# AdityaNG/Low-Cost-Hardware-Accelerated-Vision-Based-Depth-Perception-for-Real-Time-Applications

Hardware: AMD Instinct MI355X
Metric: stereo pairs/sec, KITTI 1242x375 D=128 (ms/frame at batch 1 in latency_ms_batch1) (higher is better)
Workload: dtype u8; 1 GPU; kitti_1242x375_D128_batch256_per_gpu_streamed; width=1242, height=375, disp_max=127, preset=driver(MIDDLEBURY+only_left+adaptive_mean+median), parallelism=batch-sharded x1, no data-path collective

## Files before the change

low-cost-hardware-accelerated-vision-based-depth-perception-for-real-time-applications_amd/csrc/kernels.hip:

```cpp
#include "sv_kernels.h"
#include "wave_ops.h"

#include <algorithm>
#include <atomic>

namespace sv {

thread_local LaunchHook g_launch_hook = {nullptr, nullptr};

const char *kernel_name(int id) {
    static const char *names[K_COUNT] = {"descriptor", "support_match", "support_filter", "grid_mark", "grid_dilate", "plane_fit", "triangles_raster", "dense_match", "lr_check",
                                         "delaunay_gpu", "ccl_band", "ccl_finish", "gap_rows", "gap_cols", "adaptive_mean", "median", "output"};
    return (id >= 0 && id < K_COUNT) ? names[id] : "?";
}



__device__ __forceinline__ uint32_t sad4(uint32_t a, uint32_t b, uint32_t acc) { return __builtin_amdgcn_sad_u8(a, b, acc); }

__device__ __forceinline__ uint32_t sad16(const uint4 &a, const uint4 &b) {
    uint32_t s = sad4(a.x, b.x, 0u);
    s = sad4(a.y, b.y, s);
    s = sad4(a.z, b.z, s);
    return sad4(a.w, b.w, s);
// ... 1127 lines not shown
        for (int r = 0; r < 3; r++) {
            A[r][0] = sd == 0 ? (double)pu[r] : (double)(pu[r] - pd[r]);
            A[r][1] = (double)pv[r];
            A[r][2] = 1.0;
            B[r] = (double)pd[r];
        }
        const bool ok = solve3(A, B);
        pl[3 * sd + 0] = ok ? (float)B[0] : 0.f;
        pl[3 * sd + 1] = ok ? (float)B[1] : 0.f;
        pl[3 * sd + 2] = ok ? (float)B[2] : 0.f;
    }
    const float plane_a = side == 0 ? pl[0] : pl[3], plane_b = side == 0 ? pl[1] : pl[4], plane_c = side == 0 ? pl[2] : pl[5];
    const float plane_d = side == 0 ? pl[3] : pl[0];
    const bool valid = (double)fabsf(plane_a) < 0.7 && (double)fabsf(plane_d) < 0.7;
    trirec[tbase] = make_float4(plane_a, plane_b, plane_c, valid ? 1.0f : 0.0f);
#pragma unroll
    for (int j = 0; j < 6; j++) planes[tbase * 6 + j] = pl[j];
    float tu[3], tv[3];
#pragma unroll
    for (int c = 0; c < 3; c++) {
        tu[c] = side == 0 ? (float)pu[c] : (float)(pu[c] - pd[c]);
        tv[c] = (float)pv[c];
    }
#pragma unroll
    for (int j = 0; j < 3; j++)
#pragma unroll
        for (int kk = 0; kk < j; kk++)
            if (tu[kk] > tu[j]) {
                float x = tu[j];
                tu[j] = tu[kk];
                tu[kk] = x;
                x = tv[j];
                tv[j] = tv[kk];
                tv[kk] = x;
            }
    const float A_u = tu[0], A_v = tv[0], B_u = tu[1], B_v = tv[1], C_u = tu[2], C_v = tv[2];
    float AB_a = 0, AC_a = 0, BC_a = 0;
    if ((int)A_u != (int)B_u) AB_a = (A_v - B_v) / (A_u - B_u);
    if ((int)A_u != (int)C_u) AC_a = (A_v - C_v) / (A_u - C_u);
    if ((int)B_u != (int)C_u) BC_a = (B_v - C_v) / (B_u - C_u);
    RasterRec r;
    r.a_u = (int)A_u;
    r.b_u = (int)B_u;
    r.c_u = (int)C_u;
    r.ac_a = AC_a;
    r.ac_b = A_v - AC_a * A_u;
    r.ab_a = AB_a;
    r.ab_b = A_v - AB_a * A_u;
    r.bc_a = BC_a;
    r.bc_b = B_v - BC_a * B_u;
    rrec[tbase] = r;
    ub = max(r.a_u, 0), ue = min(r.c_u, d.W);
    const float vlo = fminf(fminf(A_v, B_v), C_v), vhi = fmaxf(fmaxf(A_v, B_v), C_v);
    vb = max((int)vlo - 1, 0), ve = min((int)vhi + 2, d.H);
    }
    const bool bins = ub < ue && vb < ve;
    const int tx_lo = ub / RT_W, tx_hi = bins ? (ue - 1) / RT_W : -1, ty_lo = vb / RT_H, ty_hi = bins ? (ve - 1) / RT_H : -1;
    for (int ty = ty_lo; ty <= ty_hi; ty++)
        for (int tx = tx_lo; tx <= tx_hi; tx++) atomicAdd(&s_cnt[ty * ntx + tx], 1);
    __syncthreads();
    const size_t tb = (size_t)(pair * 2 + side) * ntile;
    for (int i = threadIdx.x; i < ntile; i += 256) {
        const int c = s_cnt[i];
        if (c > 0) s_base[i] = atomicAdd(&tile_cnt[tb + i], c);
        s_cnt[i] = 0;
    }
    __syncthreads();
    for (int ty = ty_lo; ty <= ty_hi; ty++)
        for (int tx = tx_lo; tx <= tx_hi; tx++) {
            const int tile = ty * ntx + tx;
            const int slot = s_base[tile] + atomicAdd(&s_cnt[tile], 1);
            if (slot < k.rt_cap) tile_list[(tb + tile) * RT_CAP + slot] = t;
        }
}


__global__ __launch_bounds__(256) void k_raster_tiles(KParams k, const int32_t *__restrict__ blob, const RasterRec *__restrict__ rrec, const int32_t *__restrict__ tile_cnt,
                                                      const int32_t *__restrict__ tile_list, int32_t *__restrict__ tri_id) {
    const Dims &d = k.d;
    const int pair = blockIdx.z, side = blockIdx.y;
    if (blob[pair * META_WORDS] < 3) return;
    const int ntx = (d.W + RT_W - 1) / RT_W;
    const int tx0 = (blockIdx.x % ntx) * RT_W, ty0 = (blockIdx.x / ntx) * RT_H;
    __shared__ int32_t tile[RT_H][RT_W];
    for (int i = threadIdx.x; i < RT_H * RT_W; i += 256) (&tile[0][0])[i] = -1;
    __syncthreads();
    const size_t gt = (size_t)(pair * 2 + side) * gridDim.x + blockIdx.x;
    const int listed = tile_cnt[gt];
    const bool all = listed > k.rt_cap;
    const int cnt = all ? blob[pair * META_WORDS + 2 + 2 * side] : listed;
    const int sub = threadIdx.x & 7, grp = threadIdx.x >> 3;
    const int x_end = min(tx0 + RT_W, d.W), y_end = min(ty0 + RT_H, d.H);
    const RasterRec *recs = rrec + (size_t)(pair * 2 + side) * d.max_tri;
    const int32_t *list = tile_list + gt * RT_CAP;
    int t_next = grp < cnt ? (all ? grp : list[grp]) : 0;
    RasterRec r_next = recs[t_next];
    for (int i = grp; i < cnt; i += 32) {
        const int t = t_next;
        const RasterRec r = r_next;
        if (i + 32 < cnt) {
            t_next = all ? i + 32 : list[i + 32];
            r_next = recs[t_next];
        }
        const int u_begin = max(max(r.a_u, 0), tx0), u_end = min(min(r.c_u, d.W), x_end);
        for (int base = u_begin; base < u_end; base += 8) {
            const int u = base + sub;
            int lo = 0x7FFFFFFF, hi = -0x7FFFFFFF;
            if (u < u_end) {
                const bool second = u >= r.b_u;
                const float e_a = second ? r.bc_a : r.ab_a, e_b = second ? r.bc_b : r.ab_b;
                const int v_1 = (int)(r.ac_a * (float)u + r.ac_b), v_2 = (int)(e_a * (float)u + e_b);
                lo = max(max(min(v_1, v_2), 0), ty0);
                hi = min(min(max(v_1, v_2), d.H), y_end);
                if (lo >= hi) {
                    lo = 0x7FFFFFFF;
                    hi = -0x7FFFFFFF;
                }
            }
            int32_t *p = lo < hi ? &tile[lo - ty0][u - tx0] : nullptr;
            for (int v = lo; v < hi; v++, p += RT_W) atomicMax(p, t);
        }
    }
    __syncthreads();
    int32_t *ids = tri_id + (size_t)(pair * 2 + side) * d.N;
    for (int i = threadIdx.x; i < RT_H * RT_W; i += 256) {
        const int r = i / RT_W, c = i - r * RT_W;
        if (ty0 + r < d.H && tx0 + c < d.W) map_st(ids, (uint32_t)((ty0 + r) * d.W + tx0 + c), tile[r][c]);
    }
}

void launch_triangles(const KParams &k, const SlotDev &s, int n, int max_points, hipStream_t st) {
    const int ntile = ((k.d.W + RT_W - 1) / RT_W) * ((k.d.H + RT_H - 1) / RT_H);
    const int nt = std::max(1, std::min(2 * max_points, k.d.max_tri));
    const size_t pl_lds = sizeof(int32_t) * 2 * (size_t)ntile;
    static std::atomic<size_t> pl_granted[64];
    ensure_dynamic_lds(k_planes, pl_lds, pl_granted, "plane_fit");
    SV_LAUNCH(K_PLANES, k_planes, dim3((nt + 255) / 256, 2, n), dim3(256), pl_lds, st, k, s.blob, s.trirec, s.planes, (RasterRec *)s.rrec, s.tile_cnt, s.tile_list);
    SV_LAUNCH(K_TRIANGLES, k_raster_tiles, dim3(ntile, 2, n), dim3(256), 0, st, k, s.blob, (const RasterRec *)s.rrec, s.tile_cnt, s.tile_list, s.tri_id);
}

#define DENSE_TW 512
#define DENSE_MASK_WORDS 8

template <int R>
__device__ __forceinline__ int dense_band_full(const KParams &k, int side, const uint4 own, const uint4 *pb, uint32_t vmask) {
    uint4 c[2 * R + 1];
#pragma unroll
    for (int s = 0; s <= 2 * R; s++) c[s] = pb[s];
    int key[2 * R + 1];
#pragma unroll
    for (int s = 0; s <= 2 * R; s++) {
        const int o = side ? s : 2 * R - s, ao = s < R ? R - s : s - R;
        key[s] = sad16_key(own, c[s], (int)(vmask & (((uint32_t)k.prior[ao] << 16) | (uint32_t)o)));
    }
    int bb = key[0];
#pragma unroll
    for (int s = 1; s + 1 <= 2 * R; s += 2) bb = min(bb, min(key[s], key[s + 1]));
    return bb;
}

template <bool COUNT, int MWT, int RT, bool TEX>
__device__ __forceinline__ int dense_pixel(const KParams &k, int side, int u, int v, const uint4 own, const uint4 *pu, const float4 rec, const uint32_t *mw,
                                             const uint32_t *cell, int &ncand, int (&npath)[5], const uint4 *lds_first, const uint4 *lds_last) {
    const Dims &d = k.d;
    const int MW = MWT ? MWT : d.MW, plane_radius = RT ? RT : k.plane_radius;
    if (TEX && (int)texture16(own) < k.match_texture) return -10;
    const int d_plane = (int)(rec.x * (float)u + rec.y * (float)v + rec.z);
    const int d_plane_min = max(d_plane - plane_radius, 0);
    const int d_plane_max = min(d_plane + plane_radius, d.D - 1);
    const bool valid = rec.w != 0.0f;
    const int a_lo = side ? 0 : max(u - (d.W - 3), 0), a_hi = side ? min(d.W - 3 - u, d.D - 1) : min(u - 2, d.D - 1);
    const int sgn = side ? 1 : -1;
    constexpr int KEY_NONE = 0x7FFF0000;
    int best = KEY_NONE;
    const int b_lo = max(d_plane_min, a_lo), b_hi = min(d_plane_max, a_hi);
    const bool clip = __builtin_amdgcn_ballot_w64(a_lo != 0 || a_hi != d.D - 1) != 0;
    const int band_bits = max(d_plane_max - d_plane_min + 1, 0), band_word = d_plane_min >> 5;
    const uint64_t band = (uint64_t)((1u << band_bits) - 1u) << (d_plane_min & 31);
    const uint32_t band_lo = (uint32_t)band, band_hi = (uint32_t)(band >> 32);
    uint32_t mc[DENSE_MASK_WORDS];
#pragma unroll
    for (int w = 0; w < DENSE_MASK_WORDS; w++) mc[w] = mw[w];
    if (clip) {
#pragma unroll
        for (int w = 0; w < DENSE_MASK_WORDS; w++) {
            if (w >= MW) break;
            const int lo = a_lo - 32 * w, hi = a_hi - 32 * w;
            uint32_t keep = 0;
            if (lo <= 31 && hi >= 0 && lo <= hi) {
                const int l = max(lo, 0), h = min(hi, 31);
                keep = (h == 31 ? 0xFFFFFFFFu : ((1u << (h + 1)) - 1u)) & ~((1u << l) - 1u);
            }
            mc[w] &= keep;
        }
    }
#pragma unroll
    for (int w = 0; w < DENSE_MASK_WORDS; w++) {
        if (w >= MW) break;
        if (__builtin_amdgcn_ballot_w64(mc[w] != 0u) == 0) continue;
        uint32_t m = mc[w] & ~(w == band_word ? band_lo : (w == band_word + 1 ? band_hi : 0u));
        if (COUNT) ncand += __popc(m);
        int best_w = KEY_NONE;
        while (m) {
            if (COUNT) {
                const unsigned long long act = __ballot(1);
                npath[3] += ((int)(threadIdx.x & 63) == __ffsll((long long)act) - 1) ? 1 : 0;
                npath[4]++;
            }
            const int b1 = __ffs((int)m) - 1;
            m &= m - 1;
// ... 151 lines not shown
                if (COUNT) npix++;
            }
            if (!d.sub)
                wta[(size_t)ps * d.N + (size_t)v * d.W + u] = (int16_t)out;
            else if (!(u & 1) && (u >> 1) < d.Wm && (v >> 1) < d.Hm)
                wta[(size_t)ps * d.Nm + (size_t)(v >> 1) * d.Wm + (u >> 1)] = (int16_t)out;
        }
    }
    if (COUNT) {
        count_add(counters + CNT_DENSE_CANDIDATES, ncand);
        count_add(counters + CNT_DENSE_PIXELS, npix);
        count_add(counters + CNT_DENSE_BAND_FULL, npath[0]);
        count_add(counters + CNT_DENSE_BAND_PART, npath[1]);
        count_add(counters + CNT_DENSE_BAND_SLOW, npath[2]);
        count_add(counters + CNT_DENSE_GRID_WAVE_TRIPS, npath[3]);
        count_add(counters + CNT_DENSE_GRID_LANE_TRIPS, npath[4]);
    }
}

static size_t dense_lds_bytes(const KParams &k) { return sizeof(uint4) * 2 * (size_t)dense_seg(k.d); }

template <int MWT, int RT, bool TEX>
static void launch_dense_as(const KParams &k, const SlotDev &s, const dim3 &grid, size_t shmem, hipStream_t st) {
    static std::atomic<size_t> granted[64];
    ensure_dynamic_lds(k_dense<false, MWT, RT, TEX>, shmem, granted, "dense_match");
    SV_LAUNCH(K_DENSE, (k_dense<false, MWT, RT, TEX>), grid, dim3(256), shmem, st, k, s.grad, s.blob, s.tri_id, s.trirec, s.gmaskB, s.wta, s.counters);
}

void launch_dense(const KParams &k, const SlotDev &s, int n, hipStream_t st) {
    const size_t shmem = dense_lds_bytes(k);
    const dim3 grid((k.d.W + DENSE_TW - 1) / DENSE_TW, k.d.sub ? (k.d.H + 1) / 2 : k.d.H, n);
    if (s.counters) {
        static std::atomic<size_t> granted_c[64];
        ensure_dynamic_lds(k_dense<true, 0, 0, true>, shmem, granted_c, "dense_match");
        SV_LAUNCH(K_DENSE, (k_dense<true, 0, 0, true>), grid, dim3(256), shmem, st, k, s.grad, s.blob, s.tri_id, s.trirec, s.gmaskB, s.wta, s.counters);
        return;
    }
    const int MW = k.d.MW, R = k.plane_radius;
    if (R == 3 && k.match_texture <= 0) {
        if (MW == 4) return launch_dense_as<4, 3, false>(k, s, grid, shmem, st);
        if (MW == 8) return launch_dense_as<8, 3, false>(k, s, grid, shmem, st);
        if (MW == 2) return launch_dense_as<2, 3, false>(k, s, grid, shmem, st);
        if (MW == 6) return launch_dense_as<6, 3, false>(k, s, grid, shmem, st);
    }
    if (MW == 4 && R == 3) return launch_dense_as<4, 3, true>(k, s, grid, shmem, st);
    if (MW == 8 && R == 3) return launch_dense_as<8, 3, true>(k, s, grid, shmem, st);
    if (MW == 4 && R == 2) return launch_dense_as<4, 2, true>(k, s, grid, shmem, st);
    if (MW == 8 && R == 2) return launch_dense_as<8, 2, true>(k, s, grid, shmem, st);
    if (MW == 2 && R == 2) return launch_dense_as<2, 2, true>(k, s, grid, shmem, st);
    launch_dense_as<0, 0, true>(k, s, grid, shmem, st);
}

__global__ __launch_bounds__(256) void k_lr(KParams k, const int32_t *__restrict__ blob, const int16_t *__restrict__ wta, float *__restrict__ disp,
                                            float *__restrict__ user_d2, int keep_right) {
    const Dims &d = k.d;
    const int pair = blockIdx.z;
    if (blob[pair * META_WORDS] < 3) return;
    const int u = blockIdx.x * 256 + threadIdx.x, v = blockIdx.y;
    if (u >= d.W) return;
    const int16_t *W1 = wta + (size_t)(pair * 2) * d.N, *W2 = W1 + d.N;
    const size_t row = (size_t)v * d.W;
    const float d1 = (float)W1[row + u], d2 = (float)W2[row + u];
    const float thr = (float)k.lr_threshold;
    float o1 = -10.0f, o2 = -10.0f;
    const float uw1 = d.sub ? (float)u - d1 / 2 : (float)u - d1, uw2 = d.sub ? (float)u + d2 / 2 : (float)u + d2;
    if (d1 >= 0 && uw1 >= 0 && uw1 < (float)d.W) o1 = (fabsf((float)W2[row + (int)uw1] - d1) > thr) ? -10.0f : d1;
    if (d2 >= 0 && uw2 >= 0 && uw2 < (float)d.W) o2 = (fabsf((float)W1[row + (int)uw2] - d2) > thr) ? -10.0f : d2;
    disp[(size_t)(pair * 2) * d.N + row + u] = o1;
    if (keep_right) disp[(size_t)(pair * 2 + 1) * d.N + row + u] = o2;
    if (user_d2) user_d2[(size_t)pair * d.N + row + u] = o2;
}

template <bool SUB>
__global__ __launch_bounds__(256) void k_lr2(KParams k, const int32_t *__restrict__ blob, const int16_t *__restrict__ wta, float *__restrict__ disp,
                                             float *__restrict__ user_d2, int keep_right) {
    const Dims &d = k.d;
    const int pair = blockIdx.z;
    if (blob[pair * META_WORDS] < 3) return;
    const int u = 2 * (blockIdx.x * 256 + threadIdx.x), v = blockIdx.y;
    if (u >= d.W) return;
    const size_t row = (size_t)v * d.W;
    const int16_t *W1 = wta + (size_t)(pair * 2) * d.N + row, *W2 = W1 + d.N;
    const short2 a = map_ld(reinterpret_cast<const short2 *>(W1), (uint32_t)u >> 1), b = map_ld(reinterpret_cast<const short2 *>(W2), (uint32_t)u >> 1);
    const float thr = (float)k.lr_threshold;
    float o1[2], o2[2];
#pragma unroll
    for (int j = 0; j < 2; j++) {
        const float d1 = (float)(j ? a.y : a.x), d2 = (float)(j ? b.y : b.x);
        const int uj = u + j;
        o1[j] = o2[j] = -10.0f;
        const float uw1 = SUB ? (float)uj - d1 / 2 : (float)uj - d1, uw2 = SUB ? (float)uj + d2 / 2 : (float)uj + d2;
        if (d1 >= 0 && uw1 >= 0 && uw1 < (float)d.W) o1[j] = (fabsf((float)map_ld(W2, (uint32_t)(int)uw1) - d1) > thr) ? -10.0f : d1;
        if (d2 >= 0 && uw2 >= 0 && uw2 < (float)d.W) o2[j] = (fabsf((float)map_ld(W1, (uint32_t)(int)uw2) - d2) > thr) ? -10.0f : d2;
    }
    float *D1r = disp + (size_t)(pair * 2) * d.N + row;
    map_st(reinterpret_cast<float2 *>(D1r), (uint32_t)u >> 1, make_float2(o1[0], o1[1]));
    if (keep_right) map_st(reinterpret_cast<float2 *>(D1r + d.N), (uint32_t)u >> 1, make_float2(o2[0], o2[1]));
    if (user_d2) map_st(reinterpret_cast<float2 *>(user_d2 + (size_t)pair * d.N + row), (uint32_t)u >> 1, make_float2(o2[0], o2[1]));
}

void launch_lr(const KParams &k, const SlotDev &s, int n, hipStream_t st, float *user_d2, bool keep_right) {
    if ((k.d.W & 1) == 0 && (reinterpret_cast<uintptr_t>(user_d2) & 7) == 0 && k.d.sub)
        SV_LAUNCH(K_LR, k_lr2<true>, dim3((k.d.W / 2 + 255) / 256, k.d.H, n), dim3(256), 0, st, k, s.blob, s.wta, s.disp, user_d2, keep_right ? 1 : 0);
    else if ((k.d.W & 1) == 0 && (reinterpret_cast<uintptr_t>(user_d2) & 7) == 0)
        SV_LAUNCH(K_LR, k_lr2<false>, dim3((k.d.W / 2 + 255) / 256, k.d.H, n), dim3(256), 0, st, k, s.blob, s.wta, s.disp, user_d2, keep_right ? 1 : 0);
    else
        SV_LAUNCH(K_LR, k_lr, dim3((k.d.W + 255) / 256, k.d.H, n), dim3(256), 0, st, k, s.blob, s.wta, s.disp, user_d2, keep_right ? 1 : 0);
}

__device__ __forceinline__ size_t map_offset(const Dims &d, int m, int nproc) {
    const int pair = m / nproc, side = m - pair * nproc;
    return (size_t)(pair * 2 + side) * d.N;
}

constexpr int CCL_R = 8;
constexpr int CCL_THREADS_ALONE = 1024;
constexpr int CCL_THREADS = 256;

struct CclWs {
    int4 *runs;
    int32_t *gparent;
    int32_t *total;
    int32_t *nruns;
    int32_t *boff;
    int32_t *tcount;
    int32_t *flag;
    uint64_t *bwords;
    int32_t *bbase;
    int cap, rcap, nb, nch;
};

static size_t ccl_align(size_t x) { return (x + 255) & ~(size_t)255; }

static size_t ccl_views(const KParams &k, void *ws, int maps_cap, CclWs &w) {
    w.cap = k.ccl_cap;
    w.rcap = std::max(k.d.Nm / 4, 4096);
    w.nb = (k.d.Hm + CCL_R - 1) / CCL_R;
    w.nch = (k.d.Wm + 63) / 64;
    const size_t rcap_full = (size_t)std::max(k.d.N / 4, 4096), nb_full = (size_t)(k.d.H + CCL_R - 1) / CCL_R, nch_full = (size_t)(k.d.W + 63) / 64;
    uint8_t *base = static_cast<uint8_t *>(ws);
    size_t o = 0;
    const size_t nodes = (size_t)maps_cap * rcap_full;
    w.runs = reinterpret_cast<int4 *>(base + o);
    o += ccl_align(nodes * sizeof(int4));
    w.gparent = reinterpret_cast<int32_t *>(base + o);
    o += ccl_align(nodes * 4);
    w.total = reinterpret_cast<int32_t *>(base + o);
    o += ccl_align(nodes * 4);
    w.nruns = reinterpret_cast<int32_t *>(base + o);
    o += ccl_align((size_t)maps_cap * 4);
    w.boff = reinterpret_cast<int32_t *>(base + o);
    o += ccl_align((size_t)maps_cap * nb_full * 4);
    w.tcount = reinterpret_cast<int32_t *>(base + o);
    o += ccl_align((size_t)maps_cap * nb_full * 4);
    w.flag = reinterpret_cast<int32_t *>(base + o);
    o += ccl_align((size_t)maps_cap * 4);
    w.bwords = reinterpret_cast<uint64_t *>(base + o);
    o += ccl_align((size_t)maps_cap * nb_full * 5 * nch_full * 8);
    w.bbase = reinterpret_cast<int32_t *>(base + o);
    o += ccl_align((size_t)maps_cap * nb_full * 2 * nch_full * 4);
    return o;
}

size_t ccl_ws_bytes(const KParams &k, int maps_cap) {
    CclWs w;
    return ccl_views(k, nullptr, maps_cap, w);
}

size_t ccl_lds_bytes(const KParams &k) { return (size_t)CCL_R * ((k.d.W + 63) / 64) * (3 * 8 + 4) + (size_t)k.ccl_cap * 2 * 4; }

__device__ __forceinline__ int ccl_find(const int32_t *L, int x) {
    int p = __hip_atomic_load(&L[x], __ATOMIC_RELAXED, __HIP_MEMORY_SCOPE_AGENT);
    while (p != x) {
        x = p;
        p = __hip_atomic_load(&L[x], __ATOMIC_RELAXED, __HIP_MEMORY_SCOPE_AGENT);
    }
// ... 199 lines not shown
        bw[nch + c] = Vm[c];
        bw[2 * nch + c] = Lm[c];
        bw[3 * nch + c] = Sm[rl];
        bw[4 * nch + c] = Vm[rl];
        bb[c] = base[c];
        bb[nch + c] = rowbase[rows - 1] + base[rl];
    }
}

__device__ void ccl_legacy_init_row(const KParams &k, const float *D, int32_t *L, int32_t *S, int32_t *C, int v, int lane) {
    const Dims &d = k.d;
    int carry_start = -1;
    float carry_val = -10.0f;
    for (int u0 = 0; u0 < d.W; u0 += 64) {
        const int u = u0 + lane;
        const float val = u < d.W ? D[u] : -10.0f;
        const bool valid = val >= 0;
        float left = __shfl_up(val, 1, 64);
        if (lane == 0) left = carry_val;
        const bool link = valid && left >= 0 && fabsf(val - left) <= k.speckle_sim;
        const unsigned long long brk = __ballot(!link);
        const unsigned long long upto = brk & bits_upto(lane);
        const int start = upto ? (u0 + 63 - __clzll((long long)upto)) : carry_start;
        const bool next_breaks = lane == 63 ? false : ((brk >> (lane + 1)) & 1ull) != 0;
        if (u < d.W) {
            L[u] = valid ? (int)(v * d.W + start) : -1;
            if (!(valid && start == u)) S[u] = 0;
            C[u] = 0;
            if (valid && (next_breaks || u == d.W - 1)) S[start] = u - start + 1;
        }
        carry_start = __shfl(valid ? start : -1, 63, 64);
        carry_val = __shfl(val, 63, 64);
        if (u0 + 64 < d.W) {
            const float nxt = D[u0 + 64];
            const bool cont = carry_start >= 0 && nxt >= 0 && fabsf(nxt - carry_val) <= k.speckle_sim;
            if (lane == 63 && valid && !cont) S[start] = u - start + 1;
        }
    }
}

__device__ __forceinline__ void ccl_phase_sync() {
    __builtin_amdgcn_fence(__ATOMIC_SEQ_CST, "agent");
    __syncthreads();
}

__device__ void ccl_legacy_map(const KParams &k, float *D, int32_t *label, int32_t *csize, int32_t *cnt) {
    const Dims &d = k.d;
    const int tid = threadIdx.x, nt = blockDim.x;
    const float thr = k.speckle_sim;
    for (int v = tid >> 6; v < d.H; v += nt >> 6)
        ccl_legacy_init_row(k, D + (size_t)v * d.W, label + (size_t)v * d.W, csize + (size_t)v * d.W, cnt + (size_t)v * d.W, v, tid & 63);
    ccl_phase_sync();
    for (int p = d.W + tid; p < d.N; p += nt) {
        const int u = p % d.W;
        const float c = D[p], up = D[p - d.W];
        if (!(c >= 0 && up >= 0 && fabsf(c - up) <= thr)) continue;
        if (u > 0) {
            const float cl = D[p - 1], ul = D[p - d.W - 1];
            if (cl >= 0 && ul >= 0 && fabsf(c - cl) <= thr && fabsf(up - ul) <= thr && fabsf(cl - ul) <= thr) continue;
        }
        ccl_union(label, p, p - d.W);
    }
    ccl_phase_sync();
    for (int p = tid; p < d.N; p += nt) {
        const int len = csize[p];
        if (len <= 0) continue;
        const int root = ccl_find(label, p);
        if (root != p) label[p] = root;
        atomicAdd(&cnt[root], len);
    }
    ccl_phase_sync();
    for (int p = tid; p < d.N; p += nt) {
        const int start = __hip_atomic_load(&label[p], __ATOMIC_RELAXED, __HIP_MEMORY_SCOPE_AGENT);
        if (start < 0) continue;
        const int root = __hip_atomic_load(&label[start], __ATOMIC_RELAXED, __HIP_MEMORY_SCOPE_AGENT);
        if (__hip_atomic_load(&cnt[root], __ATOMIC_RELAXED, __HIP_MEMORY_SCOPE_AGENT) < k.speckle_size) D[p] = -10.0f;
    }
}

__global__ __launch_bounds__(256) void k_ccl_border(int nproc, int epoch, const int32_t *__restrict__ blob, CclWs ws) {
    const int m = blockIdx.y;
    if (blob[(m / nproc) * META_WORDS] < 3 || ws.flag[m] == epoch) return;
    const int nch = ws.nch, nb = ws.nb;
    const int idx = blockIdx.x * 4 + (threadIdx.x >> 6), lane = threadIdx.x & 63;
    if (idx >= (nb - 1) * nch) return;
    const int b = 1 + idx / nch, c = idx - (b - 1) * nch;
    const uint64_t *bwb = ws.bwords + ((size_t)m * nb + b) * 5 * nch, *bwp = bwb - 5 * nch;
    const uint64_t L = bwb[2 * nch + c];
    if (!L) return;
    const uint64_t S0 = bwb[c], V0 = bwb[nch + c], Sp = bwp[3 * nch + c], Vp = bwp[4 * nch + c];
    const uint64_t carry = c > 0 ? (bwb[2 * nch + c - 1] >> 63) : 0ull;
    const uint64_t F = ccl_new_links(L, V0 & ~S0, Vp & ~Sp, carry);
    if (!((F >> lane) & 1ull)) return;
    const int32_t *bbb = ws.bbase + ((size_t)m * nb + b) * 2 * nch, *bbp = bbb - 2 * nch;
    const int32_t *BO = ws.boff + (size_t)m * nb;
    const int n0 = BO[b] + bbb[c], np = BO[b - 1] + bbp[nch + c];
    int32_t *GP = ws.gparent + (size_t)m * ws.rcap;
    const uint64_t upto = bits_upto(lane);
    ccl_union_halving(GP, n0 + __popcll(S0 & upto) - 1, np + __popcll(Sp & upto) - 1);
}

constexpr int CCL_SPLIT = 4;
__global__ __launch_bounds__(256) void k_ccl_total(int nproc, int epoch, int speckle_size, const int32_t *__restrict__ blob, CclWs ws) {
    const int m = blockIdx.y, b = blockIdx.x / CCL_SPLIT, part = blockIdx.x - b * CCL_SPLIT;
    if (blob[(m / nproc) * META_WORDS] < 3 || ws.flag[m] == epoch) return;
    const int T = ws.tcount[(size_t)m * ws.nb + b], off = ws.boff[(size_t)m * ws.nb + b];
    int32_t *GP = ws.gparent + (size_t)m * ws.rcap;
    int32_t *TOT = ws.total + (size_t)m * ws.rcap;
    const int4 *RUNS = ws.runs + (size_t)m * ws.rcap;
    for (int i = part * 256 + threadIdx.x; i < T; i += 256 * CCL_SPLIT) {
        const int4 r = RUNS[off + i];
        if (r.z != off + i || r.w >= speckle_size) continue;
        const int root = ccl_find_frozen(GP, off + i);
        if (root < 0) {
            GP[off + i] = CCL_LARGE;
            continue;
        }
        if (__hip_atomic_load(&TOT[root], __ATOMIC_RELAXED, __HIP_MEMORY_SCOPE_AGENT) < speckle_size) atomicAdd(&TOT[root], r.w);
        GP[off + i] = root;
    }
}

__global__ __launch_bounds__(256) void k_ccl_apply(KParams k, int nproc, int epoch, const int32_t *__restrict__ blob, float *__restrict__ disp, CclWs ws, int32_t *__restrict__ label,
                                                   int32_t *__restrict__ csize, int32_t *__restrict__ cnt) {
    const Dims &d = k.d;
    const int m = blockIdx.y;
    if ((int)blockIdx.x == ws.nb * CCL_SPLIT) {
        if (threadIdx.x == 0) ws.nruns[m] = 0;
        if (blob[(m / nproc) * META_WORDS] < 3 || ws.flag[m] != epoch) return;
        const size_t off = map_offset(d, m, nproc);
        ccl_legacy_map(k, disp + off, label + off, csize + off, cnt + off);
        return;
    }
    const int b = blockIdx.x / CCL_SPLIT, part = blockIdx.x - b * CCL_SPLIT;
    if (blob[(m / nproc) * META_WORDS] < 3 || ws.flag[m] == epoch) return;
    const int T = ws.tcount[(size_t)m * ws.nb + b], off = ws.boff[(size_t)m * ws.nb + b];
    const int32_t *GP = ws.gparent + (size_t)m * ws.rcap, *TOT = ws.total + (size_t)m * ws.rcap;
    const int4 *RUNS = ws.runs + (size_t)m * ws.rcap;
    float *D = disp + map_offset(d, m, nproc);
    for (int i = part * 256 + threadIdx.x; i < T; i += 256 * CCL_SPLIT) {
        const int4 r = RUNS[off + i];
        if (r.y >= k.speckle_size) continue;
        const int root = ccl_find_frozen(GP, off + i);
        if (root < 0 || TOT[root] >= k.speckle_size) continue;
        for (int q = 0; q < r.y; q++) D[r.x + q] = -10.0f;
    }
}

void launch_speckle(const KParams &k, const SlotDev &s, int n, int nproc, hipStream_t st) {
    const int maps = n * nproc;
    CclWs ws;
    ccl_views(k, s.ccl_ws, s.cap * 2, ws);
    const size_t lds = ccl_lds_bytes(k);
    const int epoch = (int)(++s.ccl_epoch & 0x3FFFFFFFu) + 1;
    static std::atomic<size_t> granted[64], granted_alone[64];
    if ((size_t)ws.nb * maps <= 256) {
        ensure_dynamic_lds(k_ccl_band<CCL_THREADS_ALONE>, lds, granted_alone, "ccl_band");
        SV_LAUNCH(K_CCL_BAND, k_ccl_band<CCL_THREADS_ALONE>, dim3(ws.nb, maps), dim3(CCL_THREADS_ALONE), lds, st, k, nproc, epoch, s.blob, s.disp, ws);
    } else {
        ensure_dynamic_lds(k_ccl_band<CCL_THREADS>, lds, granted, "ccl_band");
        SV_LAUNCH(K_CCL_BAND, k_ccl_band<CCL_THREADS>, dim3(ws.nb, maps), dim3(CCL_THREADS), lds, st, k, nproc, epoch, s.blob, s.disp, ws);
    }
    if (ws.nb > 1) SV_LAUNCH(K_CCL_FINISH, k_ccl_border, dim3(((ws.nb - 1) * ws.nch + 3) / 4, maps), dim3(256), 0, st, nproc, epoch, s.blob, ws);
    SV_LAUNCH(K_CCL_FINISH, k_ccl_total, dim3(ws.nb * CCL_SPLIT, maps), dim3(256), 0, st, nproc, epoch, k.speckle_size, s.blob, ws);
    int32_t *cnt = reinterpret_cast<int32_t *>(s.tmp);
    SV_LAUNCH(K_CCL_FINISH, k_ccl_apply, dim3(ws.nb * CCL_SPLIT + 1, maps), dim3(256), 0, st, k, nproc, epoch, s.blob, s.disp, ws, s.tri_id, s.csize, cnt);
}

__device__ __forceinline__ float gap_value(float d1, float d2) {
    return fabsf(d1 - d2) < 3.0f ? (d1 + d2) / 2 : (d2 < d1 ? d2 : d1);
}

#define SV_MAX_LINE_WORDS 128

#define GAPR_THREADS 256
__global__ __launch_bounds__(GAPR_THREADS) void k_gap_rows(KParams k, int nproc, const int32_t *__restrict__ blob, float *__restrict__ disp) {
    const Dims &d = k.d;
    const int m = blockIdx.y;
    if (blob[(m / nproc) * META_WORDS] < 3) return;
    float *D = disp + map_offset(d, m, nproc) + (size_t)blockIdx.x * d.W;
    const int lane = threadIdx.x & 63, wave = threadIdx.x >> 6, nw = GAPR_THREADS / 64;
    const int nch = (d.W + 63) / 64;
    __shared__ unsigned long long mw[SV_MAX_LINE_WORDS];
    __shared__ int prevb[SV_MAX_LINE_WORDS], nextb[SV_MAX_LINE_WORDS];
    for (int c = wave; c < nch; c += nw) {
        const int u = c * 64 + lane;
        const float val = u < d.W ? map_ld(D, (uint32_t)u) : -1.0f;
        const unsigned long long b = __ballot(val >= 0);
        if (lane == 0) mw[c] = b;
    }
    __syncthreads();
    if (wave == 0) {
        int carry = -1;
        for (int c0 = 0; c0 < nch; c0 += 64) {
            const int c = c0 + lane;
            const unsigned long long w = c < nch ? mw[c] : 0ull;
            int last = w ? c * 64 + 63 - __clzll((long long)w) : -1;
#pragma unroll
            for (int o = 1; o < 64; o <<= 1) {
                const int t = __shfl_up(last, o, 64);
                if (lane >= o) last = max(last, t);
            }
            int excl = __shfl_up(last, 1, 64);
            if (lane == 0) excl = -1;
            if (c < nch) prevb[c] = max(excl, carry);
            carry = max(carry, __shfl(last, 63, 64));
        }
    } else if (wave == 1) {
        int carry = 0x7FFFFFFF;
        for (int c0 = ((nch - 1) / 64) * 64; c0 >= 0; c0 -= 64) {
            const int c = c0 + lane;
            const unsigned long long w = c < nch ? mw[c] : 0ull;
            int first = w ? c * 64 + __ffsll((long long)w) - 1 : 0x7FFFFFFF;
#pragma unroll
            for (int o = 1; o < 64; o <<= 1) {
                const int t = __shfl_down(first, o, 64);
                if (lane + o < 64) first = min(first, t);
            }
            int excl = __shfl_down(first, 1, 64);
            if (lane == 63) excl = 0x7FFFFFFF;
            const int nb = min(excl, carry);
            if (c < nch) nextb[c] = nb == 0x7FFFFFFF ? -1 : nb;
            carry = min(carry, __shfl(first, 0, 64));
        }
    }
    __syncthreads();
    const int gw = k.gap_width;
    for (int c = wave; c < nch; c += nw) {
        const int u = c * 64 + lane;
        const unsigned long long w = mw[c];
        if (u >= d.W || ((w >> lane) & 1ull)) continue;
        const unsigned long long below = w & ((1ull << lane) - 1ull);
        const unsigned long long above = lane == 63 ? 0ull : (w >> (lane + 1));
        const int pl = below ? c * 64 + 63 - __clzll((long long)below) : prevb[c];
        const int nr = above ? u + __ffsll((long long)above) : nextb[c];
        if (pl >= 0 && nr >= 0) {
            if (nr - pl - 1 <= gw) map_st(D, (uint32_t)u, gap_value(map_ld(D, (uint32_t)pl), map_ld(D, (uint32_t)nr)));
        } else if (k.add_corners) {
            if (pl < 0 && nr >= 0) {
                if (u >= nr - gw) map_st(D, (uint32_t)u, map_ld(D, (uint32_t)nr));
            } else if (nr < 0 && pl >= 0) {
                if (u <= pl + gw) map_st(D, (uint32_t)u, map_ld(D, (uint32_t)pl));
            }
        }
    }
}

void launch_gap_rows(const KParams &k, const SlotDev &s, int n, int nproc, hipStream_t st) {
    SV_LAUNCH(K_GAP_ROWS, k_gap_rows, dim3(k.d.H, n * nproc), dim3(GAPR_THREADS), 0, st, k, nproc, s.blob, s.disp);
}

#define GAPC_THREADS 256
__global__ __launch_bounds__(GAPC_THREADS) void k_gap_cols(KParams k, int nproc, const int32_t *__restrict__ blob, float *__restrict__ disp) {
    const Dims &d = k.d;
    const int m = blockIdx.y;
    if (blob[(m / nproc) * META_WORDS] < 3) return;
    float *D = disp + map_offset(d, m, nproc);
    const int lane = threadIdx.x & 63, wave = threadIdx.x >> 6;
    const int u = blockIdx.x * 64 + lane;
    extern __shared__ unsigned long long cmask[];
    const int nw = (d.H + 63) / 64;
    const bool live = u < d.W;
    for (int w = wave; w < nw; w += GAPC_THREADS / 64) {
        unsigned long long word = 0;
        const int vend = min(64, d.H - w * 64);
        const float *col = D + (size_t)(w * 64) * d.W + (live ? u : 0);
        for (int b0 = 0; b0 < vend; b0 += 16) {
            float val[16];
#pragma unroll
            for (int j = 0; j < 16; j++) val[j] = col[(size_t)min(b0 + j, vend - 1) * d.W];
#pragma unroll
            for (int j = 0; j < 16; j++) word |= (unsigned long long)(live && b0 + j < vend && val[j] >= 0) << (b0 + j);
        }
        cmask[w * 64 + lane] = word;
    }
    __syncthreads();
    if (!live) return;
    const int gw = k.gap_width;
    for (int w = wave; w < nw; w += GAPC_THREADS / 64) {
        const unsigned long long word = cmask[w * 64 + lane];
        const int vend = min(64, d.H - w * 64);
        unsigned long long inval = ~word & (vend == 64 ? ~0ull : ((1ull << vend) - 1ull));
        while (inval) {
            const int b = __ffsll((long long)inval) - 1;
            inval &= inval - 1;
            const int v = w * 64 + b;
            int pv = -1;
            {
                unsigned long long below = word & ((1ull << b) - 1ull);
                int ww = w;
                for (;;) {
                    if (below) {
                        pv = ww * 64 + 63 - __clzll((long long)below);
                        break;
                    }
                    if (--ww < 0) break;
                    below = cmask[ww * 64 + lane];
                }
            }
            int nv = -1;
            {
                unsigned long long above = b == 63 ? 0ull : (word >> (b + 1)) << (b + 1);
                int ww = w;
                for (;;) {
                    if (above) {
                        nv = ww * 64 + __ffsll((long long)above) - 1;
                        break;
                    }
                    if (++ww >= nw) break;
                    above = cmask[ww * 64 + lane];
                }
            }
            if (pv >= 0 && nv >= 0) {
                if (nv - pv - 1 <= gw) D[(size_t)v * d.W + u] = gap_value(D[(size_t)pv * d.W + u], D[(size_t)nv * d.W + u]);
            } else if (k.add_corners) {
                if (pv < 0 && nv >= 0) {
                    if (v >= nv - gw) D[(size_t)v * d.W + u] = D[(size_t)nv * d.W + u];
                } else if (nv < 0 && pv >= 0) {
// ... 410 lines not shown
```

Baseline: 48900 pairs/s.

## Micro-optimize raster tiles, LR check, and gap-row kernels

```diff
diff --git a/low-cost-hardware-accelerated-vision-based-depth-perception-for-real-time-applications_amd/csrc/kernels.hip b/low-cost-hardware-accelerated-vision-based-depth-perception-for-real-time-applications_amd/csrc/kernels.hip
--- a/low-cost-hardware-accelerated-vision-based-depth-perception-for-real-time-applications_amd/csrc/kernels.hip
+++ b/low-cost-hardware-accelerated-vision-based-depth-perception-for-real-time-applications_amd/csrc/kernels.hip
@@ -1233,8 +1233,10 @@
     if (blob[pair * META_WORDS] < 3) return;
     const int ntx = (d.W + RT_W - 1) / RT_W;
     const int tx0 = (blockIdx.x % ntx) * RT_W, ty0 = (blockIdx.x / ntx) * RT_H;
-    __shared__ int32_t tile[RT_H][RT_W];
-    for (int i = threadIdx.x; i < RT_H * RT_W; i += 256) (&tile[0][0])[i] = -1;
+    __shared__ __align__(16) int32_t tile[RT_H][RT_W];
+    static_assert(RT_H * RT_W == 2 * 4 * 256, "two 16-byte stores per thread clear the tile");
+    reinterpret_cast<int4 *>(&tile[0][0])[threadIdx.x] = make_int4(-1, -1, -1, -1);
+    reinterpret_cast<int4 *>(&tile[0][0])[threadIdx.x + 256] = make_int4(-1, -1, -1, -1);
     __syncthreads();
     const size_t gt = (size_t)(pair * 2 + side) * gridDim.x + blockIdx.x;
     const int listed = tile_cnt[gt];
@@ -1254,29 +1256,46 @@
             r_next = recs[t_next];
         }
         const int u_begin = max(max(r.a_u, 0), tx0), u_end = min(min(r.c_u, d.W), x_end);
-        for (int base = u_begin; base < u_end; base += 8) {
+        int col = 4 * (u_begin + sub - tx0 - ty0 * RT_W);
+        for (int base = u_begin; base < u_end; base += 8, col += 4 * 8) {
             const int u = base + sub;
-            int lo = 0x7FFFFFFF, hi = -0x7FFFFFFF;
+            int lo = ty0, n = 0;
             if (u < u_end) {
                 const bool second = u >= r.b_u;
                 const float e_a = second ? r.bc_a : r.ab_a, e_b = second ? r.bc_b : r.ab_b;
                 const int v_1 = (int)(r.ac_a * (float)u + r.ac_b), v_2 = (int)(e_a * (float)u + e_b);
                 lo = max(max(min(v_1, v_2), 0), ty0);
-                hi = min(min(max(v_1, v_2), d.H), y_end);
-                if (lo >= hi) {
-                    lo = 0x7FFFFFFF;
-                    hi = -0x7FFFFFFF;
-                }
-            }
-            int32_t *p = lo < hi ? &tile[lo - ty0][u - tx0] : nullptr;
-            for (int v = lo; v < hi; v++, p += RT_W) atomicMax(p, t);
+                n = min(min(max(v_1, v_2), d.H), y_end) - lo;
+            }
+            int32_t *p = reinterpret_cast<int32_t *>(reinterpret_cast<char *>(&tile[0][0]) + (lo * (4 * RT_W) + col));
+            for (; n >= 2; n -= 2, p += 2 * RT_W) {
+                atomicMax(p, t);
+                atomicMax(p + RT_W, t);
+            }
+            if (n > 0) atomicMax(p, t);
         }
     }
     __syncthreads();
     int32_t *ids = tri_id + (size_t)(pair * 2 + side) * d.N;
-    for (int i = threadIdx.x; i < RT_H * RT_W; i += 256) {
-        const int r = i / RT_W, c = i - r * RT_W;
-        if (ty0 + r < d.H && tx0 + c < d.W) map_st(ids, (uint32_t)((ty0 + r) * d.W + tx0 + c), tile[r][c]);
+    static_assert(RT_W == 64 && RT_H == 32, "32 column pairs x 8 rows per pass, four passes");
+    const int cp = 2 * (threadIdx.x & 31), x = tx0 + cp;
+    const int r0 = threadIdx.x >> 5, rows = d.H - ty0 - r0;
+    if (x >= d.W) return;
+    const int32_t *src = &tile[r0][cp];
+    const uint32_t at = (uint32_t)((ty0 + r0) * d.W + x);
+    if ((d.W & 1) == 0) {
+#pragma unroll
+        for (int j = 0; j < RT_H / 8; j++)
+            if (8 * j < rows) map_st(reinterpret_cast<int2 *>(ids), (at + (uint32_t)(8 * j * d.W)) >> 1, *reinterpret_cast<const int2 *>(src + 8 * j * RT_W));
+    } else {
+        const bool second = x + 1 < d.W;
+#pragma unroll
+        for (int j = 0; j < RT_H / 8; j++)
+            if (8 * j < rows) {
+                const int2 t = *reinterpret_cast<const int2 *>(src + 8 * j * RT_W);
+                map_st(ids, at + (uint32_t)(8 * j * d.W), t.x);
+                if (second) map_st(ids, at + (uint32_t)(8 * j * d.W) + 1u, t.y);
+            }
     }
 }
 
@@ -1594,8 +1613,23 @@
     const size_t row = (size_t)v * d.W;
     const int16_t *W1 = wta + (size_t)(pair * 2) * d.N + row, *W2 = W1 + d.N;
     const short2 a = map_ld(reinterpret_cast<const short2 *>(W1), (uint32_t)u >> 1), b = map_ld(reinterpret_cast<const short2 *>(W2), (uint32_t)u >> 1);
+    float o1[2], o2[2];
+    if constexpr (!SUB) {
+        const int thr = min(k.lr_threshold, 1 << 20);
+        const bool some = thr >= 0;
+        const uint32_t span = some ? 2u * (uint32_t)thr : 0u;
+#pragma unroll
+        for (int j = 0; j < 2; j++) {
+            const int d1 = j ? a.y : a.x, d2 = j ? b.y : b.x;
+            const int p1 = u + j - d1, p2 = u + j + d2;
+            bool keep1 = false, keep2 = false;
+            if (d1 >= 0 && (unsigned)p1 < (unsigned)d.W) keep1 = some && (uint32_t)((int)map_ld(W2, (uint32_t)p1) - d1 + thr) <= span;
+            if (d2 >= 0 && (unsigned)p2 < (unsigned)d.W) keep2 = some && (uint32_t)((int)map_ld(W1, (uint32_t)p2) - d2 + thr) <= span;
+            o1[j] = keep1 ? (float)d1 : -10.0f;
+            o2[j] = keep2 ? (float)d2 : -10.0f;
+        }
+    } else {
     const float thr = (float)k.lr_threshold;
-    float o1[2], o2[2];
 #pragma unroll
     for (int j = 0; j < 2; j++) {
         const float d1 = (float)(j ? a.y : a.x), d2 = (float)(j ? b.y : b.x);
@@ -1604,6 +1638,7 @@
         const float uw1 = SUB ? (float)uj - d1 / 2 : (float)uj - d1, uw2 = SUB ? (float)uj + d2 / 2 : (float)uj + d2;
         if (d1 >= 0 && uw1 >= 0 && uw1 < (float)d.W) o1[j] = (fabsf((float)map_ld(W2, (uint32_t)(int)uw1) - d1) > thr) ? -10.0f : d1;
         if (d2 >= 0 && uw2 >= 0 && uw2 < (float)d.W) o2[j] = (fabsf((float)map_ld(W1, (uint32_t)(int)uw2) - d2) > thr) ? -10.0f : d2;
+    }
     }
     float *D1r = disp + (size_t)(pair * 2) * d.N + row;
     map_st(reinterpret_cast<float2 *>(D1r), (uint32_t)u >> 1, make_float2(o1[0], o1[1]));
@@ -1969,7 +2004,7 @@
     const int m = blockIdx.y;
     if (blob[(m / nproc) * META_WORDS] < 3 || ws.flag[m] == epoch) return;
     const int nch = ws.nch, nb = ws.nb;
-    const int idx = blockIdx.x * 4 + (threadIdx.x >> 6), lane = threadIdx.x & 63;
+    const int idx = blockIdx.x * 4 + __builtin_amdgcn_readfirstlane(threadIdx.x >> 6), lane = threadIdx.x & 63;
     if (idx >= (nb - 1) * nch) return;
     const int b = 1 + idx / nch, c = idx - (b - 1) * nch;
     const uint64_t *bwb = ws.bwords + ((size_t)m * nb + b) * 5 * nch, *bwp = bwb - 5 * nch;
@@ -2066,10 +2101,10 @@
     const int m = blockIdx.y;
     if (blob[(m / nproc) * META_WORDS] < 3) return;
     float *D = disp + map_offset(d, m, nproc) + (size_t)blockIdx.x * d.W;
-    const int lane = threadIdx.x & 63, wave = threadIdx.x >> 6, nw = GAPR_THREADS / 64;
+    const int lane = threadIdx.x & 63, wave = __builtin_amdgcn_readfirstlane(threadIdx.x >> 6), nw = GAPR_THREADS / 64;
     const int nch = (d.W + 63) / 64;
     __shared__ unsigned long long mw[SV_MAX_LINE_WORDS];
-    __shared__ int prevb[SV_MAX_LINE_WORDS], nextb[SV_MAX_LINE_WORDS];
+    __shared__ int2 ends[SV_MAX_LINE_WORDS];
     for (int c = wave; c < nch; c += nw) {
         const int u = c * 64 + lane;
         const float val = u < d.W ? map_ld(D, (uint32_t)u) : -1.0f;
@@ -2090,7 +2125,7 @@
             }
             int excl = __shfl_up(last, 1, 64);
             if (lane == 0) excl = -1;
-            if (c < nch) prevb[c] = max(excl, carry);
+            if (c < nch) ends[c].x = max(excl, carry);
             carry = max(carry, __shfl(last, 63, 64));
         }
     } else if (wave == 1) {
@@ -2107,20 +2142,25 @@
             int excl = __shfl_down(first, 1, 64);
             if (lane == 63) excl = 0x7FFFFFFF;
             const int nb = min(excl, carry);
-            if (c < nch) nextb[c] = nb == 0x7FFFFFFF ? -1 : nb;
+            if (c < nch) ends[c].y = nb == 0x7FFFFFFF ? -1 : nb;
             carry = min(carry, __shfl(first, 0, 64));
         }
     }
     __syncthreads();
     const int gw = k.gap_width;
+    const unsigned long long lt = (1ull << lane) - 1ull, gt = ~((lt << 1) | 1ull);
+    const uint32_t lt_lo = (uint32_t)lt, lt_hi = (uint32_t)(lt >> 32), gt_lo = (uint32_t)gt, gt_hi = (uint32_t)(gt >> 32);
+    const uint32_t me_lo = ~(lt_lo | gt_lo), me_hi = ~(lt_hi | gt_hi);
     for (int c = wave; c < nch; c += nw) {
         const int u = c * 64 + lane;
         const unsigned long long w = mw[c];
-        if (u >= d.W || ((w >> lane) & 1ull)) continue;
-        const unsigned long long below = w & ((1ull << lane) - 1ull);
-        const unsigned long long above = lane == 63 ? 0ull : (w >> (lane + 1));
-        const int pl = below ? c * 64 + 63 - __clzll((long long)below) : prevb[c];
-        const int nr = above ? u + __ffsll((long long)above) : nextb[c];
+        const int2 e = ends[c];
+        const uint32_t w_lo = (uint32_t)w, w_hi = (uint32_t)(w >> 32);
+        if (u >= d.W || ((w_lo & me_lo) | (w_hi & me_hi))) continue;
+        const unsigned long long below = ((unsigned long long)(w_hi & lt_hi) << 32) | (w_lo & lt_lo);
+        const unsigned long long above = ((unsigned long long)(w_hi & gt_hi) << 32) | (w_lo & gt_lo);
+        const int pl = below ? (c * 64 + 63) ^ __clzll((long long)below) : e.x;
+        const int nr = above ? (c * 64 - 1) + __ffsll((long long)above) : e.y;
         if (pl >= 0 && nr >= 0) {
             if (nr - pl - 1 <= gw) map_st(D, (uint32_t)u, gap_value(map_ld(D, (uint32_t)pl), map_ld(D, (uint32_t)nr)));
         } else if (k.add_corners) {
```

After: 49740 pairs/s (median of 6 runs). +1.7%, better.
